# jixinya/EAMM

Measured on AMD Instinct MI355X. Metric: 256x256 frames/sec (dense-motion + generator forward), higher is better.
Workload: dtype f32; 1 GPU; 256x256, 10 keypoints, batch=16 synthetic frames per GPU per step, source encoded once per clip (BASELINE.json configs[2]); parallelism=frame-sharded x1

## Files before the change

eamm_amd/_lib.py:

```python
from __future__ import annotations

import ctypes as C
import os

_HERE = os.path.dirname(os.path.abspath(__file__))
LIB_PATH = os.path.join(_HERE, "libeamm_hip.so")

ABI_VERSION = 6

EAMM_OK = 0
ERR_ARG, ERR_STATE, ERR_KEY, ERR_HIP, ERR_NUMERIC = -1, -2, -3, -4, -5


class EammConfig(C.Structure):
    _fields_ = [
        ("num_channels", C.c_int32), ("num_kp", C.c_int32), ("block_expansion", C.c_int32),
        ("max_features", C.c_int32), ("num_down_blocks", C.c_int32), ("num_bottleneck_blocks", C.c_int32),
        ("estimate_occlusion_map", C.c_int32), ("dm_block_expansion", C.c_int32),
        ("dm_max_features", C.c_int32), ("dm_num_blocks", C.c_int32), ("dm_inv_scale", C.c_int32),
        ("kp_variance", C.c_float), ("height", C.c_int32), ("width", C.c_int32),
        ("max_frames", C.c_int32), ("max_sources", C.c_int32),
    ]


# ... 96 lines not shown
    "eamm_bn_backward_apply": (C.c_int, [C.c_void_p, C.c_void_p, C.c_void_p, C.c_void_p, C.c_int, C.c_int, C.c_int, C.c_void_p,
                                         C.c_void_p]),
    "eamm_bn_apply": (C.c_int, [C.c_void_p, C.c_void_p, C.c_void_p, C.c_void_p, C.c_int, C.c_int, C.c_int, C.c_void_p,
                                C.c_void_p]),
    "eamm_bn_last_error": (C.c_char_p, []),
    "eamm_profile_enable": (C.c_int, [C.c_void_p, C.c_int]),
    "eamm_profile_read": (C.c_int, [C.c_void_p, C.POINTER(C.c_double), C.c_int, C.POINTER(C.c_int64),
                                    C.POINTER(C.c_int64), C.c_int]),
    "eamm_op_conv": (C.c_int, [C.c_int, C.c_void_p, C.c_int, C.c_void_p, C.c_int, C.c_int, C.c_int, C.c_int,
                               C.c_int, C.c_void_p, C.c_void_p, C.c_int, C.c_int, C.c_int, C.c_int, C.c_int, C.c_void_p,
                               C.c_int, C.c_int, C.c_void_p, C.c_int, C.POINTER(C.c_float), C.c_void_p]),
    "eamm_op_conv_ex": (C.c_int, [C.c_int, C.c_void_p, C.c_int, C.c_void_p, C.c_int, C.c_int, C.c_int, C.c_int,
                                  C.c_int, C.c_void_p, C.c_void_p, C.c_int, C.c_int, C.c_int, C.c_int, C.c_int, C.c_void_p,
                                  C.c_int, C.c_int, C.c_void_p, C.c_int, C.POINTER(C.c_float), C.c_void_p, C.c_void_p, C.c_void_p,
                                  C.c_void_p, C.c_void_p, C.c_int, C.c_int, C.c_void_p]),
    "eamm_op_wino_transform": (C.c_int, [C.c_int, C.c_void_p, C.c_void_p, C.c_void_p, C.c_int, C.c_int, C.c_int, C.c_int, C.c_int,
                                         C.c_void_p, C.c_void_p]),
    "eamm_op_warp_ex": (C.c_int, [C.c_int, C.c_void_p, C.c_void_p, C.c_void_p, C.c_int, C.c_int, C.c_int, C.c_int, C.c_int,
                                  C.c_int, C.c_int, C.c_void_p, C.c_int, C.POINTER(C.c_float), C.c_void_p, C.c_void_p, C.c_void_p,
                                  C.c_void_p]),
    "eamm_set_training": (C.c_int, [C.c_void_p, C.c_int]),
    "eamm_train_num_sites": (C.c_int, [C.c_void_p]),
    "eamm_train_site_name": (C.c_char_p, [C.c_void_p, C.c_int]),
    "eamm_train_max_channels": (C.c_int, [C.c_void_p]),
    "eamm_train_begin": (C.c_int, [C.c_void_p, C.c_void_p, C.c_int, C.c_void_p, C.c_void_p, C.c_void_p, C.c_void_p,
                                   C.POINTER(EammBnSite), C.c_int, C.c_float, C.c_float, C.c_int, C.c_void_p, C.POINTER(EammOutputs),
                                   C.c_void_p]),
    "eamm_train_next": (C.c_int, [C.c_void_p, C.POINTER(C.c_int)]),
    "eamm_op_warp": (C.c_int, [C.c_int, C.c_void_p, C.c_void_p, C.c_void_p, C.c_int, C.c_int, C.c_int, C.c_int, C.c_int,
                               C.c_int, C.c_int, C.c_void_p, C.c_int, C.POINTER(C.c_float), C.c_void_p]),
# ... 145 lines not shown
```

eamm_amd/csrc/api_common.h:

```cpp
#pragma once
#include "../../include/eamm_hip.h"
#include "kernels.h"

#include <algorithm>
#include <cmath>
#include <cstdarg>
#include <cstdio>
#include <cstdlib>
#include <cstring>
#include <map>
#include <string>
#include <vector>

namespace eamm {

inline thread_local std::string g_create_error;

namespace {

struct HostTensor {
    std::vector<int64_t> shape;
    std::vector<float> data;
    size_t numel() const {
        size_t n = 1;
// ... 175 lines not shown
    std::copy(b.begin(), b.end(), pad.begin());
    return upload(c, dst, pad);
}

int upload_conv_image(CtxBase* c, float** dst, const HostConv& f, const int* map, int cin_packed, int BN, LayerMode mode,
                      bool swizzle) {
    const bool phase = mode == MODE_PHASE || mode == MODE_PHASES;
    std::vector<float> packed(conv_packed_elems(phase ? 4 : f.kh * f.kw, cin_packed, f.Cout, BN, phase ? 4 : 1));
    if (mode == MODE_PHASES)
        conv_pack_phases_host(f.w.data(), f.Cout, f.Cin, map, cin_packed, BN, swizzle, packed.data());
    else
        conv_pack_host(f.w.data(), f.Cout, f.Cin, f.kh, f.kw, map, cin_packed, BN, phase, swizzle, packed.data());
    return upload(c, dst, packed);
}

int pack_conv(CtxBase* c, const HostConv& f, const int* map, int C0_packed, int C1_packed, LayerMode mode, int dma_cfg,
              ConvLayer* L, int BN = 0) {
    const bool phase = mode == MODE_PHASE || mode == MODE_PHASES;
    L->kh = f.kh;
    L->kw = f.kw;
    L->phase = phase;
    L->C0 = C0_packed;
    L->C1 = C1_packed;
    L->Cout = f.Cout;
    L->BM = 128;
    L->BN = BN ? BN : conv_tile_n(f.Cout);
    L->dma_cfg = dma_cfg;
    if (dma_cfg > 0 && !conv_dma_tile(dma_cfg, &L->BM, &L->BN)) return fail(c, EAMM_ERR_ARG, "unknown dma tile %d", dma_cfg);
    L->ntiles = (f.Cout + L->BN - 1) / L->BN;
    L->nchunks = (phase ? 4 : f.kh * f.kw) * ((C0_packed + C1_packed) / CONV_BK);
// ... 31 lines not shown
    if (tile == 4)
        wino4_pack_host(f.w.data(), f.Cout, f.Cin, L->BN, packed.data());
    else
        wino_pack_host(f.w.data(), f.Cout, f.Cin, L->BN, packed.data());
    if (int rc = upload(c, &L->u, packed)) return rc;
    if (split_planes && tile == 4 && f.Cin % (4 * CONV_BK) == 0) {
        std::vector<float> planes(wino4_split_packed_elems(f.Cout, f.Cin, L->BN));
        wino4_pack_split_host(f.w.data(), f.Cout, f.Cin, L->BN, reinterpret_cast<uint16_t*>(planes.data()));
        if (int rc = upload(c, &L->u3, planes)) return rc;
    }
    return upload_bias(c, &L->bias, f.b, (size_t)L->ntiles * L->BN);
}

int build_layer(CtxBase* c, const std::vector<FoldSpec>& parts, int ks, int C0_real, int C0_packed, int C1_real,
                int C1_packed, ConvLayer* L, LayerMode mode = MODE_PLAIN, std::vector<float>* row_bias = nullptr,
                int dma_cfg = 0, float** w_swizzled = nullptr, int w_swizzled_bn = 0) {
    if (mode != MODE_PLAIN && mode != MODE_ROWSPLIT) return fail(c, EAMM_ERR_ARG, "build_layer: plain or row-split layers only");
    HostConv f;
    if (int rc = fold_conv(c, parts, ks, C0_real + C1_real, &f)) return rc;
    if (mode == MODE_ROWSPLIT) {
        std::vector<float> rb = to_rowsplit(&f);
        if (row_bias) row_bias->swap(rb);
    }
    const std::vector<int> map = channel_map(C0_real, C0_packed, C1_real, C1_packed);
    if (int rc = pack_conv(c, f, map.data(), C0_packed, C1_packed, MODE_PLAIN, dma_cfg, L)) return rc;
    if (!w_swizzled) return EAMM_OK;
    return upload_conv_image(c, w_swizzled, f, map.data(), C0_packed + C1_packed, w_swizzled_bn ? w_swizzled_bn : L->BN,
                             MODE_PLAIN, true);
}

int build_set(CtxBase* c, const std::vector<FoldSpec>& parts, int C0_real, int C0_packed, int C1_real, int C1_packed,
              LayerSet* S, LayerMode mode, bool patch_split_planes = false) {
    HostConv f;
    int rc = fold_conv(c, parts, 3, C0_real + C1_real, &f);
    if (rc) return rc;
    const std::vector<int> map = channel_map(C0_real, C0_packed, C1_real, C1_packed);
    if ((rc = pack_conv(c, f, map.data(), C0_packed, C1_packed, mode, 0, &S->base))) return rc;
    const int Cout = S->base.Cout;
    int cfg = 0;
    if (Cout % 256 == 0) cfg = c->dma_cfg_n256;
// ... 142 lines not shown
```

eamm_amd/csrc/conv_col7.hip:

```cpp
#include "conv_common.h"

#include <algorithm>
#include <cstdlib>

namespace eamm {

typedef __attribute__((address_space(3))) void* lds_ptr_t;

namespace {
constexpr int CT = 16;
constexpr int CPR = CT + 6;
constexpr int CPIX = CPR * CT;
constexpr int CWAVES = 8;
constexpr int CMAXCH = 2;
}

struct Col7Args {
    const float* in;
    unsigned in_bytes, w_bytes;
    int C, B, H, W;
    int tiles_x, tiles_y, tiles;
    const float* w;
    float* out;
    const float* bias;
// ... 328 lines not shown
                static_for<4>([&](auto ic) {
                    constexpr int i = decltype(ic)::value;
                    if (12 * nh + 4 * g + i < PS) dst[4 * g + i] = acc[g][i];
                    acc[g][i] = 0.f;
                });
            });
            __syncthreads();
            col7_gather_tile(p, scratch, Carry, bias_r, b, ty0, tx0, tid);
        }
        asm volatile("s_waitcnt vmcnt(0)" ::: "memory");
        __syncthreads();
        cur = nxt;
    }
}

struct Col7sArgs {
    const float* in0;
    const float* in1;
    unsigned in0_bytes, in1_bytes, w_bytes;
    int C0, C1, B, H, W;
    int tiles_x, tiles_y;
    const float* w;
    float* out;
    int PS;
};

template <int NT>
__global__ __launch_bounds__(CWAVES * 64) void conv_col7s_kernel(const Col7sArgs p) {
    constexpr int BK = CONV_BK;
    constexpr int A_STAGE = CPIX * BK;
// ... 123 lines not shown
    a.W = W;
    a.tiles_x = (W + CT - 1) / CT;
    a.tiles_y = (H + CT - 1) / CT;
    a.w = w_swizzled;
    a.out = out;
    a.PS = pixel_stride;
    constexpr size_t lds = sizeof(float) * (2 * CPIX * CONV_BK + 2 * 3 * 32 * CONV_BK);
    static_assert(lds <= 160 * 1024, "LDS budget");
    static lds_once_mask configured{0};
    if (hipError_t e = ensure_dynamic_lds(conv_col7s_kernel<3>, lds, &configured); e != hipSuccess) return e;
    note_mfma_flops(2.0 * a.tiles_x * a.tiles_y * B * (CT * CT) * 7.0 * (ntile32 * 32) * (C0 + C1));
    hipLaunchKernelGGL(conv_col7s_kernel<3>, dim3(a.tiles_x * a.tiles_y * B), dim3(CWAVES * 64), lds, stream, a);
    return hipGetLastError();
}

static hipError_t col7_launch_impl(const float* in, int C, int B, int H, int W, const float* w_swizzled, float* out, const float* bias,
                                   float* final_out, hipStream_t stream) {
    const bool fused = final_out != nullptr;
    if (C % CONV_BK || C / CONV_BK > CMAXCH || C < CONV_BK) return hipErrorInvalidValue;
    Col7Args a{};
    a.in = in;
    const size_t ib = (size_t)B * H * W * C * 4, wb = (size_t)(C / CONV_BK) * 7 * 32 * CONV_BK * 4;
    if (ib >= 0xFFFFFFF0ull) return hipErrorInvalidValue;
    a.in_bytes = (unsigned)ib;
    a.w_bytes = (unsigned)wb;
    a.C = C;
    a.B = B;
    a.H = H;
    a.W = W;
    a.tiles_x = (W + CT - 1) / CT;
    a.tiles_y = (H + CT - 1) / CT;
    a.tiles = B * a.tiles_x * a.tiles_y;
// ... 6 lines not shown
    a.dbg = dbg;
#else
    a.dbg = 0;
#endif
    const size_t lds = wb + sizeof(float) * (2 * CPIX * CONV_BK + (fused ? 2 * CT * 6 * 21 : 0));
    if (lds > 160 * 1024) return hipErrorInvalidValue;
    static lds_once_mask configured{0}, configured_fused{0};
    if (hipError_t e = fused ? ensure_dynamic_lds(conv_col7_kernel<true>, 160 * 1024, &configured_fused)
                             : ensure_dynamic_lds(conv_col7_kernel<false>, 160 * 1024, &configured);
        e != hipSuccess)
        return e;
    int dev = 0, cus = 256;
    (void)hipGetDevice(&dev);
    (void)hipDeviceGetAttribute(&cus, hipDeviceAttributeMultiprocessorCount, dev);
    const int blocks = std::min(fused ? B * a.tiles_y : a.tiles, cus);
    static const bool mfma4 = knob_int("EAMM_FINAL_MFMA4", 1) != 0;
    if (fused && mfma4) {
        static lds_once_mask configured_q{0};
        note_mfma_flops(2.0 * a.tiles * (CT * CT) * 7.0 * 24 * C);
        if (hipError_t e = ensure_dynamic_lds(conv_col7q_kernel<8>, 160 * 1024, &configured_q); e != hipSuccess) return e;
        hipLaunchKernelGGL(conv_col7q_kernel<8>, dim3(blocks), dim3(CWAVES * 64), lds, stream, a);
        return hipGetLastError();
    }
    note_mfma_flops(2.0 * a.tiles * (CT * CT) * 7.0 * 32 * C);
    if (fused)
        hipLaunchKernelGGL(conv_col7_kernel<true>, dim3(blocks), dim3(CWAVES * 64), lds, stream, a);
    else
        hipLaunchKernelGGL(conv_col7_kernel<false>, dim3(blocks), dim3(CWAVES * 64), lds, stream, a);
    return hipGetLastError();
}

hipError_t conv_col7_launch(const float* in, int C, int B, int H, int W, const float* w_swizzled, float* out,
                            hipStream_t stream) {
    return col7_launch_impl(in, C, B, H, W, w_swizzled, out, nullptr, nullptr, stream);
}

hipError_t conv_col7_fused_launch(const float* in, int C, int B, int H, int W, const float* w_swizzled, const float* bias,
                                  float* out_nchw, hipStream_t stream) {
    if (!bias || !out_nchw) return hipErrorInvalidValue;
    return col7_launch_impl(in, C, B, H, W, w_swizzled, nullptr, bias, out_nchw, stream);
}

}
```

eamm_amd/csrc/eamm_api.hip:

```cpp
#include "eamm_ctx.h"

namespace {

void expected_keys(const eamm_ctx* c, std::vector<std::string>* keys) {
    auto block = [&](const std::string& p) { block_keys(p, keys); };
    const std::string dm = "dense_motion_network.";
    for (int i = 0; i < c->nb; ++i) block(dm + "hourglass.encoder.down_blocks." + std::to_string(i));
    for (int i = 0; i < c->nb; ++i) block(dm + "hourglass.decoder.up_blocks." + std::to_string(i));
    if (c->nb > 0) {
        keys->push_back(dm + "mask.weight");
        keys->push_back(dm + "mask.bias");
        if (c->cfg.estimate_occlusion_map) {
            keys->push_back(dm + "occlusion.weight");
            keys->push_back(dm + "occlusion.bias");
        }
        if (c->cfg.dm_inv_scale != 1) keys->push_back(dm + "down.weight");
    }
    block("first");
    for (int i = 0; i < c->nd; ++i) block("down_blocks." + std::to_string(i));
    for (int i = 0; i < c->nd; ++i) block("up_blocks." + std::to_string(i));
    for (int i = 0; i < c->cfg.num_bottleneck_blocks; ++i) {
        const std::string r = "bottleneck.r" + std::to_string(i);
        for (const char* s : {".conv1.weight", ".conv1.bias", ".conv2.weight", ".conv2.bias", ".norm1.weight",
                              ".norm1.bias", ".norm1.running_mean", ".norm1.running_var", ".norm2.weight",
// ... 378 lines not shown
            if ((rc = build_wino4_rect(c, p + ".conv", p + ".norm", ci, ci, &c->w4down[i]))) return rc;
        }
    }
    c->up.resize(c->nd);
    for (int i = 0; i < c->nd; ++i) {
        const std::string p = "up_blocks." + std::to_string(i);
        const int ci = i == 0 ? c->Cb : c->up_c[i - 1];
        if ((rc = build_set(c, {{p + ".conv", nm(p + ".norm")}}, ci, ci, 0, 0, &c->up[i], MODE_PHASE, true))) return rc;
    }
    if (c->Cimg > 3) {
        if ((rc = build_layer(c, {{"final", ""}}, 7, c->up_c.back(), c->up_c.back(), 0, 0, &c->final_conv))) return rc;
    } else {
        std::vector<float> fb;
        const bool col7_ok = c->col7 && c->up_c.back() % 32 == 0 && c->up_c.back() <= 64;
        if ((rc = build_layer(c, {{"final", ""}}, 7, c->up_c.back(), c->up_c.back(), 0, 0, &c->final_conv,
                              MODE_ROWSPLIT, &fb, 0, col7_ok ? &c->final_w_swz : nullptr)))
            return rc;
        if (c->final_conv.Cout != 21) return fail(c, EAMM_ERR_KEY, "final.weight must have 3 output channels");
        if ((rc = upload(c, &c->final_bias, fb))) return rc;
    }
    {
        std::vector<float> aa((size_t)c->Cpl * 169, 0.f);
        if (g.dm_inv_scale != 1) {
            const HostTensor* t = find(c, dm + "down.weight");
            if (!t || (int)t->numel() != c->Cpl * 169) return fail(c, EAMM_ERR_KEY, "%sdown.weight must be [%d,1,13,13]", dm.c_str(), c->Cimg);
            aa = t->data;
        }
        if ((rc = upload(c, &c->aa_w, aa))) return rc;
    }

    const size_t S = g.max_sources, F = g.max_frames;
// ... 253 lines not shown
```

eamm_amd/csrc/eamm_ctx.h:

```cpp
#pragma once
#include "../../include/eamm_hip.h"
#include "api_common.h"

#include <functional>

using namespace eamm;

struct PassProfile {
    static constexpr int NSTAGE = 22;
    static constexpr int MAXCHAIN = 4;
    static constexpr int NMARK = 8;
    static constexpr int NSUB = 64;
    static constexpr int PROF_CALLS = 256;
    struct Call {
        int n = 0, nchain = 0, sub = 0;
        bool complete = false;
        double flops = 0, flops_bneck = 0, stage_flops[NMARK] = {0};
    };
    bool on = false;
    std::vector<hipEvent_t> events;
    std::vector<hipEvent_t> chain_ev;
    std::vector<Call> calls;
    int used = 0;
    hipEvent_t *ev = nullptr, *cev = nullptr;
// ... 61 lines not shown
    bool wino4_variant_pinned = false;
    int cus = 256;
    float* wino_v = nullptr;
    float* wino_z = nullptr;
    size_t wino_z_elems = 0;
    int wino_min_m = 49152;
    int wino4_min_m = 0;
    std::vector<float*> pre_s, pre_t;
    float* aa_w = nullptr;
    float* head_bias = nullptr;
    int head_nc = 0;
    float* head_w_swz = nullptr;
    float* final_bias = nullptr;
    float* final_part = nullptr;
    float* final_w_swz = nullptr;
    int col7 = 1;
    int final_fused = 1;
    int final_fused_min_rows = 128;
    int head_col7_min_tiles = 128;

    float *feat = nullptr, *src_small = nullptr, *src_full = nullptr;
    float* src_nhwc = nullptr;
    std::vector<float*> enc_tmp;
    float* kp_rec = nullptr;
    int* bad_flag = nullptr;
    float* hg_in = nullptr;
    std::vector<float*> e_buf, u_buf;
    float *logits = nullptr, *deformation = nullptr, *occlusion = nullptr;
    float *xa = nullptr, *xb = nullptr, *act = nullptr, *tmp = nullptr;
    std::vector<float*> up_buf;
// ... 72 lines not shown
```

eamm_amd/csrc/eamm_forward.hip:

```cpp
#include "eamm_ctx.h"
#include <mutex>

namespace {
constexpr int POOL_MAXDEV = 64, POOL_MAXCHAIN = 15;
std::mutex g_pool_mu;
hipStream_t g_pool[POOL_MAXDEV][POOL_MAXCHAIN] = {};
std::mutex g_pool_lease[POOL_MAXDEV];

}

hipStream_t chain_stream(int device, int k) {
    if (device < 0 || device >= POOL_MAXDEV || k < 0 || k >= POOL_MAXCHAIN) return nullptr;
    std::lock_guard<std::mutex> lock(g_pool_mu);
    if (!g_pool[device][k] && hipStreamCreateWithFlags(&g_pool[device][k], hipStreamNonBlocking) != hipSuccess) g_pool[device][k] = nullptr;
    return g_pool[device][k];
}

FrameView make_view(const eamm_ctx* c, int f0, int n, int ns_call, int slab, const float* kd_val, const float* kd_jac,
                    const float* ks_val, const float* ks_jac, const eamm_outputs* o) {
    FrameView v;
    const size_t F = (size_t)f0, K = c->K;
    const size_t HW = (size_t)c->H * c->W, hw = (size_t)c->h * c->w, hwf = (size_t)c->hf * c->wf;
    const size_t sf = ns_call > 1 ? F : 0;
    v.n = n;
// ... 310 lines not shown
}

int stage_final(eamm_ctx* c, const FrameView& v, hipStream_t s) {
    const float* in = v.up_buf[c->nd - 1];
    ConvIO io = conv_for(v, in, c->H, c->W, ACT_NONE, v.final_part);
    if (c->Cimg > 3) {
        io.act = ACT_SIGMOID;
        io.nchw = 1;
        io.out = v.out.prediction;
        HIP_TRY(c, conv_launch(c->final_conv, io, s));
        return EAMM_OK;
    }
    ConvLayer fl = c->final_conv;
    fl.Cout = 32;
    if (final_is_fused(c, v.n)) {
        HIP_TRY(c, conv_col7_fused_launch(in, fl.C0, v.n, c->H, c->W, c->final_w_swz, c->final_bias, v.out.prediction, s));
    } else {
        if (c->final_w_swz && fl.BN == 32)
            HIP_TRY(c, conv_col7_launch(in, fl.C0, v.n, c->H, c->W, c->final_w_swz, v.final_part, s));
        else
            HIP_TRY(c, conv_launch(fl, io, s));
        HIP_TRY(c, final_shift_sum_launch(v.final_part, c->final_bias, v.n, c->H, c->W, v.out.prediction, s));
    }
    if (v.out.frames_u8) HIP_TRY(c, to_u8_launch(v.out.prediction, v.n, c->H, c->W, v.out.frames_u8, s));
    return EAMM_OK;
}

static int forward_view(eamm_ctx* c, const FrameView& v, hipStream_t s, int chain, bool chained) {
    PassProfile& p = c->prof;
    const bool direct = bottleneck_form(c, v.n) == 0;
    int rc;
// ... 217 lines not shown
    return pass_chains(c, n);
}
int eamm_last_stream_set(const eamm_ctx* c) { return c ? c->last_streams : EAMM_ERR_ARG; }
int eamm_describe_plan(const eamm_ctx* c, int n, char* buf, int cap) {
    if (!c || n <= 0 || n > c->cfg.max_frames || !c->finalized) return EAMM_ERR_ARG;
    const int pc = pass_chains(c, n), nk = pc > 1 ? n / pc : n;
    const int form = bottleneck_form(c, nk), bc = pc > 1 ? pc : bottleneck_chains(c, n);
    std::string enc = "[";
    for (int i = 0; i < c->nb; ++i)
        enc += std::string(i ? ", " : "") + (enc_level_wino4(c, i, nk) ? "\"wino4\"" : "\"direct\"");
    enc += "]";
    char tmp[1024];
    const int len = snprintf(tmp, sizeof tmp,
                             "{\"frames\": %d, \"pass_chains\": %d, \"frames_per_chain\": %d, \"bottleneck_form\": %d, \"bottleneck_chains\": %d, "
                             "\"wino4_groups\": %d, \"wino4_variant\": %d, \"hg_encoder\": %s, \"final\": \"%s\", "
                             "\"side_streams\": %d, \"experiments_build\": %d}",
                             n, pc, nk, form, bc, (form == 4 && pc == 1 && bc == 1) ? wino4_groups(c, n) : 1, wino4_variant_for(c, n), enc.c_str(),
                             final_is_fused(c, nk) ? "col7q fused" : "col7 + shift-sum", (int)c->pool_streams.size(),
                             eamm_build_experiments());
    if (buf && cap > 0) {
        const int m = std::min(len, cap - 1);
        std::memcpy(buf, tmp, (size_t)m);
        buf[m] = 0;
    }
    return len;
}

}
```

eamm_amd/csrc/eamm_op_conv.hip:

```cpp
#include "op_common.h"

namespace {

struct ConvOp {
    const float *in0, *in1;
    int C0, C1, B, Hin, Win, up;
    const float *w, *b;
    int Cout, kh, kw, act, pool;
    const float* resid;
    int splitk, tile_n;
    float* out;
    int iters;
    float* avg_ms;
    const float *pre_s, *pre_t;
    float* out2;
    const float *s2, *t2;
    int nchw, split_n;
    const char* name;
    hipStream_t s;
};

const char* conv_refusal(const ConvOp& a) {
    const bool staged = a.tile_n == 0 || a.tile_n == 32 || a.tile_n == 64 || a.tile_n == 128;
    const bool gemm = staged || (a.tile_n > 1000 && a.tile_n <= 1005);
    const bool wino = a.tile_n >= 2000 && a.tile_n < 2200;
    const bool shape_ok = (a.kh == 3 && a.kw == 3) || (a.kh == 7 && a.kw == 7) || (a.kh == 7 && a.kw == 1) ||
                          (a.kh == 1 && a.kw == 1 && staged && !a.up);
    if (!a.in0 || !a.w || !a.b || !a.out || !shape_ok || a.C0 % CONV_BK || a.C1 % CONV_BK || (a.up && (a.kh != 3 || a.kw != 3)))
        return "bad argument";
    if ((a.pre_s != nullptr) != (a.pre_t != nullptr)) return "pre_scale and pre_shift come together";
    if (a.pre_s && !wino) return "pre_scale / pre_shift belong to the Winograd input transform (tile codes 2000, 21xx)";
    const bool second = a.out2 || a.s2 || a.t2;
    if ((second || a.nchw || a.split_n) && !gemm)
        return "out2 / scale2 / shift2 / nchw / split_n belong to the implicit GEMM (tile codes 0, 32, 64, 128, 1001..1005)";
    if (a.split_n < 0 || (a.nchw != 0 && a.nchw != 1)) return "bad nchw / split_n";
    if ((a.s2 != nullptr) != (a.t2 != nullptr) || (a.s2 && !a.out2)) return "scale2 and shift2 come together, with out2";
    if (a.out2 && !a.s2 && a.split_n == 0) return "out2 needs scale2 and shift2";
    if (!op_aligned16(a.pre_s) || !op_aligned16(a.pre_t) || !op_aligned16(a.out2) || !op_aligned16(a.s2) || !op_aligned16(a.t2))
        return "pre_scale, pre_shift, out2, scale2 and shift2 must be 16-byte aligned";
    if (a.pool && (a.resid || a.nchw || a.out2 || a.split_n))
        return "pool does not combine with resid, nchw, out2 or split_n (the pooled epilogue has none of them)";
    if (a.split_n > 0 && (!a.out2 || a.resid || a.nchw || a.Cout <= a.split_n || a.Cout > a.split_n + 4))
        return "split_n needs out2, no resid / pool / nchw, and split_n < Cout <= split_n + 4";
    return nullptr;
}

HostConv op_weights(const ConvOp& a, int Cin, bool with_bias = true) {
    HostConv f;
    f.Cout = a.Cout;
    f.Cin = Cin;
    f.kh = a.kh;
    f.kw = a.kw;
    f.w.assign(a.w, a.w + (size_t)a.Cout * Cin * a.kh * a.kw);
    if (with_bias) f.b.assign(a.b, a.b + a.Cout);
    return f;
}

int op_conv_final(OpBuffers* t, const ConvOp& a) {
    if (a.kh != 7 || a.kw != 7 || a.Cout != 3 || a.act != 2 || a.up || a.pool || a.resid || a.C1 || a.C0 % 32 || a.C0 > 64 || a.C0 < 32)
        return fail(t, EAMM_ERR_ARG, "%s: unsupported fused final-layer configuration", a.name);
    HostConv f = op_weights(a, a.C0);
    const std::vector<float> bias = to_rowsplit(&f);
    float *w = nullptr, *b = nullptr;
    int rc = upload_conv_image(t, &w, f, nullptr, a.C0, conv_tile_n(f.Cout), MODE_PLAIN, true);
    if (rc || (rc = upload(t, &b, bias))) return rc;
    auto fused_final = [&]() { return conv_col7_fused_launch(a.in0, a.C0, a.B, a.Hin, a.Win, w, b, a.out, a.s); };
    HIP_TRY(t, fused_final());
    HIP_TRY(t, time_launches(a.s, a.iters, a.avg_ms, fused_final));
    return EAMM_OK;
}

int op_conv_col7(OpBuffers* t, const ConvOp& a) {
    const bool streamed = a.tile_n == 4001;
    const int bn = streamed ? 96 : 32;
    if (a.kh != 7 || a.kw != 1 || a.up || a.pool || a.resid || a.splitk > 1 || a.Cout != bn || a.act != 0 || a.C0 % 32 || a.C1 % 32 ||
        (!streamed && (a.C1 || a.C0 > 64)))
        return fail(t, EAMM_ERR_ARG, "%s: unsupported column-patch configuration", a.name);
    float* w = nullptr;
    if (int rc = upload_conv_image(t, &w, op_weights(a, a.C0 + a.C1, false), nullptr, a.C0 + a.C1, bn, MODE_PLAIN, true)) return rc;
    auto col7 = [&]() {
        return streamed ? conv_col7s_launch(a.in0, a.C0, a.in1, a.C1, a.B, a.Hin, a.Win, w, 3, a.out, 96, a.s)
// ... 72 lines not shown
    io.resid = a.resid;
    io.nchw = a.nchw;
    io.out2 = a.out2;
    io.s2 = a.s2;
    io.t2 = a.t2;
    io.split_n = a.split_n;
    if (io.partial_cap && (rc = dev_alloc(t, &io.partial, io.partial_cap))) return rc;
    auto gemm = [&]() { return conv_launch(L, io, a.s, a.splitk); };
    HIP_TRY(t, gemm());
    HIP_TRY(t, time_launches(a.s, a.iters, a.avg_ms, gemm));
    return EAMM_OK;
}

int op_conv_run(OpBuffers* t, const ConvOp& a) {
    int rc;
    if (a.tile_n == 4002) rc = op_conv_final(t, a);
    else if (a.tile_n == 4000 || a.tile_n == 4001) rc = op_conv_col7(t, a);
    else if (a.tile_n == 3000 || a.tile_n == 3003 || a.tile_n == 3004) rc = op_conv_patch(t, a);
    else if (a.tile_n >= 2000 && a.tile_n < 2200) rc = op_conv_wino(t, a);
    else rc = op_conv_gemm(t, a);
    if (rc) return rc;
    HIP_TRY(t, hipStreamSynchronize(a.s));
    return EAMM_OK;
}

int op_conv_call(int device, ConvOp a, void* stream_) {
    if (const char* why = conv_refusal(a)) return fail(nullptr, EAMM_ERR_ARG, "%s: %s", a.name, why);
    DeviceGuard guard(device);
    if (guard.status != hipSuccess) return fail(nullptr, EAMM_ERR_HIP, "hipSetDevice failed");
    a.s = reinterpret_cast<hipStream_t>(stream_);
    OpBuffers t(device, a.s);
// ... 29 lines not shown
    return op_conv_call(device,
                        ConvOp{in0, in1, C0, C1, B, Hin, Win, up, w_host, b_host, Cout, kh, kw, act, pool, resid, splitk, tile_n, out, iters,
                               avg_ms, pre_scale, pre_shift, out2, scale2, shift2, nchw, split_n, "eamm_op_conv_ex", nullptr},
                        stream_);
}

int eamm_op_conv(int device, const float* in0, int C0, const float* in1, int C1, int B, int Hin, int Win, int up,
                 const float* w_host, const float* b_host, int Cout, int kh, int kw, int act, int pool,
                 const float* resid, int splitk, int tile_n, float* out, int iters, float* avg_ms, void* stream_) {
    return op_conv_call(device,
                        ConvOp{in0, in1, C0, C1, B, Hin, Win, up, w_host, b_host, Cout, kh, kw, act, pool, resid, splitk, tile_n, out, iters,
                               avg_ms, nullptr, nullptr, nullptr, nullptr, nullptr, 0, 0, "eamm_op_conv", nullptr},
                        stream_);
}

int eamm_op_wino_transform(int device, const float* x, const float* scale, const float* shift, int B, int H, int W, int C, int tile,
                           float* V, void* stream_) {
    const bool tile_ok = tile == 2 || tile == 4;
    OP_ENTRY(!x || !V || !tile_ok || B < 1 || H < 1 || W < 1 || C < 1 || H % tile || W % tile || (C & 3) ||
                 (scale != nullptr) != (shift != nullptr) || !op_aligned16(x) || !op_aligned16(V) || !op_aligned16(scale) ||
                 !op_aligned16(shift) || !op_count_ok((tile + 2) * (tile + 2), (long long)B * (H / tile) * (W / tile), C),
             "eamm_op_wino_transform: bad argument");
    OP_DONE(tile == 4 ? wino4_transform_launch(x, scale, shift, B, H, W, C, V, s) : wino_transform_launch(x, scale, shift, B, H, W, C, V, s),
            "eamm_op_wino_transform");
}

int eamm_op_warp_ex(int device, const float* feat, const float* deformation, const float* occlusion, int n, int ns, int hf, int wf, int C,
                    int h, int w, float* out, int iters, float* avg_ms, float* out2, const float* scale2, const float* shift2,
                    void* stream_) {
    return op_warp_call("eamm_op_warp_ex", device, feat, deformation, occlusion, n, ns, hf, wf, C, h, w, out, out2, scale2, shift2, iters,
// ... 11 lines not shown
```

eamm_amd/csrc/kernels.h:

```cpp
#pragma once
#include <hip/hip_runtime.h>
#include <stddef.h>
#include <stdint.h>

namespace eamm {

constexpr int CONV_BK = 32;
constexpr int CONV_LDK = CONV_BK + 4;
inline size_t round64(size_t n) { return (n + 63) / 64 * 64; }
constexpr int KP_STRIDE = 8;

enum Act { ACT_NONE = 0, ACT_RELU = 1, ACT_SIGMOID = 2 };

void note_mfma_flops(double flops);
double take_mfma_flops();
double total_mfma_flops();

long long knob_int(const char* name, long long dflt);
int knobs_json(char* buf, int cap);

struct ConvArgs {
    const float* in0;
    const float* in1;
    int C0, C1;
// ... 68 lines not shown
size_t patch_packed_elems(int Cin_packed, int Cout);
size_t patch_poly_packed_elems(int Cin_packed, int Cout);
void patch_poly_pack_host(const float* w_oihw_3x3, int Cout, int Cin, const int* cin_map, int cin_packed, float* dst);
size_t patch_poly_split_packed_elems(int Cin_packed, int Cout);
void patch_poly_pack_split_host(const float* w_oihw_3x3, int Cout, int Cin, const int* cin_map, int cin_packed, uint16_t* dst);
hipError_t patch_poly_launch(const PatchLayer& L, const float* in0, const float* in1, int B, int H, int W, int act,
                             float* out, hipStream_t stream, int splits = 1, float* partial = nullptr, size_t partial_cap = 0);
int patch_poly_splits(const PatchLayer& L, int B, int H, int W, int max_splits, int cus);
void patch_pack_host(const float* w_oihw_3x3, int Cout, int Cin, const int* cin_map, int cin_packed, float* dst);
hipError_t patch_phase_launch(const PatchLayer& L, const float* in0, const float* in1, int B, int H, int W, int act,
                              float* out, hipStream_t stream);

hipError_t conv_col7_launch(const float* in, int C, int B, int H, int W, const float* w_swizzled, float* out,
                            hipStream_t stream);
hipError_t conv_col7_fused_launch(const float* in, int C, int B, int H, int W, const float* w_swizzled, const float* bias,
                                  float* out_nchw, hipStream_t stream);

hipError_t conv_col7s_launch(const float* in0, int C0, const float* in1, int C1, int B, int H, int W, const float* w_swizzled,
                             int ntile32, float* out, int pixel_stride, hipStream_t stream);

struct WinoLayer {
    int Cin = 0, Cout = 0, BN = 128, ntiles = 0;
    int tile = 2;
    float* u = nullptr;
    float* u3 = nullptr;
    float* bias = nullptr;
};
size_t wino_packed_elems(int Cout, int Cin, int BN);
void wino_pack_host(const float* w_oihw, int Cout, int Cin, int BN, float* dst);
hipError_t wino_transform_launch(const float* x, const float* s, const float* t, int B, int H, int W, int C, float* V,
                                 hipStream_t stream);
// ... 233 lines not shown
```

include/eamm_hip.h:

```cpp
#ifndef EAMM_HIP_H_
#define EAMM_HIP_H_

#include <stddef.h>
#include <stdint.h>

#ifdef __cplusplus
extern "C" {
#endif

#define EAMM_ABI_VERSION 6

typedef enum eamm_status {
    EAMM_OK = 0,
    EAMM_ERR_ARG = -1,
    EAMM_ERR_STATE = -2,
    EAMM_ERR_KEY = -3,
    EAMM_ERR_HIP = -4,
    EAMM_ERR_NUMERIC = -5
} eamm_status;

typedef struct eamm_ctx eamm_ctx;

typedef struct eamm_config {
    int32_t num_channels;
// ... 202 lines not shown
#define EAMM_NSTAGE 22
int eamm_profile_enable(eamm_ctx* ctx, int on);
int eamm_profile_read(eamm_ctx* ctx, double* stage_ms, int nstage, int64_t* calls, int64_t* frames, int reset);


int eamm_op_conv(int device, const float* in0, int C0, const float* in1, int C1, int B, int Hin, int Win, int up,
                 const float* weight_host, const float* bias_host, int Cout, int kh, int kw,
                 int act, int pool, const float* resid, int splitk, int tile_n, float* out, int iters,
                 float* avg_ms, void* stream);

int eamm_op_conv_ex(int device, const float* in0, int C0, const float* in1, int C1, int B, int Hin, int Win, int up,
                    const float* weight_host, const float* bias_host, int Cout, int kh, int kw,
                    int act, int pool, const float* resid, int splitk, int tile_n, float* out, int iters,
                    float* avg_ms, const float* pre_scale, const float* pre_shift, float* out2, const float* scale2,
                    const float* shift2, int nchw, int split_n, void* stream);

int eamm_op_wino_transform(int device, const float* x, const float* scale, const float* shift, int B, int H, int W, int C, int tile,
                           float* V, void* stream);

int eamm_op_one_euro(int device, const float* x, int T, int E, float mincutoff, float beta, float dcutoff, float freq, float scale,
                     float* out, float* state, int resume, void* stream);

int64_t eamm_op_mfcc_frames(int64_t n_samples, int pad);
int eamm_op_mfcc(int device, const float* pcm, int64_t n_samples, int n_clips, int64_t clip_stride, int pad, float* out, void* stream);

int eamm_op_resize_aa(int device, const uint8_t* in, int n, int H, int W, int C, const double* taps_y, int ry, const double* taps_x,
                      int rx, uint8_t* out, void* stream);
int eamm_op_similarity_warp(int device, const uint8_t* in, int n, int H, int W, int C, const double* maps, int mode, void* out,
                            void* stream);
int eamm_op_emotion_augment(int device, const float* aligned, int64_t n_src, int64_t t0, int count, int flip, const double* rot,
// ... 127 lines not shown
```

Before: 4391 frames/s.

## Run fused final 7x7 conv on split-bf16 MFMA with pre-split weight planes

```diff
diff --git a/eamm_amd/_lib.py b/eamm_amd/_lib.py
--- a/eamm_amd/_lib.py
+++ b/eamm_amd/_lib.py
@@ -134,6 +134,8 @@
                                   C.c_int, C.c_void_p, C.c_void_p, C.c_int, C.c_int, C.c_int, C.c_int, C.c_int, C.c_void_p,
                                   C.c_int, C.c_int, C.c_void_p, C.c_int, C.POINTER(C.c_float), C.c_void_p, C.c_void_p, C.c_void_p,
                                   C.c_void_p, C.c_void_p, C.c_int, C.c_int, C.c_void_p]),
+    "eamm_final_split_planes_elems": (C.c_size_t, [C.c_int]),
+    "eamm_final_split_planes": (C.c_int, [C.c_void_p, C.c_int, C.c_void_p, C.c_void_p]),
     "eamm_op_wino_transform": (C.c_int, [C.c_int, C.c_void_p, C.c_void_p, C.c_void_p, C.c_int, C.c_int, C.c_int, C.c_int, C.c_int,
                                          C.c_void_p, C.c_void_p]),
     "eamm_op_warp_ex": (C.c_int, [C.c_int, C.c_void_p, C.c_void_p, C.c_void_p, C.c_int, C.c_int, C.c_int, C.c_int, C.c_int,
diff --git a/eamm_amd/csrc/api_common.h b/eamm_amd/csrc/api_common.h
--- a/eamm_amd/csrc/api_common.h
+++ b/eamm_amd/csrc/api_common.h
@@ -213,6 +213,12 @@
     return upload(c, dst, packed);
 }
 
+int upload_col7_split(CtxBase* c, float** dst, const HostConv& f, const int* map, int cin_packed) {
+    std::vector<float> planes(col7_split_packed_elems(cin_packed));
+    col7_pack_split_host(f.w.data(), f.Cout, f.Cin, map, cin_packed, reinterpret_cast<uint16_t*>(planes.data()));
+    return upload(c, dst, planes);
+}
+
 int pack_conv(CtxBase* c, const HostConv& f, const int* map, int C0_packed, int C1_packed, LayerMode mode, int dma_cfg,
               ConvLayer* L, int BN = 0) {
     const bool phase = mode == MODE_PHASE || mode == MODE_PHASES;
@@ -274,7 +280,7 @@
 
 int build_layer(CtxBase* c, const std::vector<FoldSpec>& parts, int ks, int C0_real, int C0_packed, int C1_real,
                 int C1_packed, ConvLayer* L, LayerMode mode = MODE_PLAIN, std::vector<float>* row_bias = nullptr,
-                int dma_cfg = 0, float** w_swizzled = nullptr, int w_swizzled_bn = 0) {
+                int dma_cfg = 0, float** w_swizzled = nullptr, int w_swizzled_bn = 0, float** w_col7_split = nullptr) {
     if (mode != MODE_PLAIN && mode != MODE_ROWSPLIT) return fail(c, EAMM_ERR_ARG, "build_layer: plain or row-split layers only");
     HostConv f;
     if (int rc = fold_conv(c, parts, ks, C0_real + C1_real, &f)) return rc;
@@ -284,6 +290,8 @@
     }
     const std::vector<int> map = channel_map(C0_real, C0_packed, C1_real, C1_packed);
     if (int rc = pack_conv(c, f, map.data(), C0_packed, C1_packed, MODE_PLAIN, dma_cfg, L)) return rc;
+    if (w_col7_split)
+        if (int rc = upload_col7_split(c, w_col7_split, f, map.data(), C0_packed + C1_packed)) return rc;
     if (!w_swizzled) return EAMM_OK;
     return upload_conv_image(c, w_swizzled, f, map.data(), C0_packed + C1_packed, w_swizzled_bn ? w_swizzled_bn : L->BN,
                              MODE_PLAIN, true);
diff --git a/eamm_amd/csrc/conv_col7.hip b/eamm_amd/csrc/conv_col7.hip
--- a/eamm_amd/csrc/conv_col7.hip
+++ b/eamm_amd/csrc/conv_col7.hip
@@ -2,6 +2,7 @@
 
 #include <algorithm>
 #include <cstdlib>
+#include <cstring>
 
 namespace eamm {
 
@@ -366,6 +367,146 @@
     }
 }
 
+namespace {
+constexpr int SG = 16;
+constexpr int S_WBLK = 2 * PS * 16;
+constexpr int S_WGROUP = 7 * 3 * S_WBLK;
+constexpr int S_WBYTES = (CMAXCH * 2 * S_WGROUP + 1023) / 1024 * 1024;
+constexpr int S_ROWS = CPR;
+constexpr int S_F32 = S_ROWS * 1024;
+constexpr int S_OCT = CPIX * 16;
+constexpr int S_PLANE = 2 * S_OCT;
+constexpr int S_PSTAGE = 3 * S_PLANE;
+constexpr int S_LDS = S_WBYTES + S_F32 + 2 * S_PSTAGE + 2 * CARRY * 4;
+static_assert(S_LDS <= 160 * 1024, "LDS budget");
+static_assert(CT * CT * PS * 4 <= S_PSTAGE, "the tile's partial products fit a consumed plane stage");
+static_assert(CPR <= 3 * CWAVES, "at most three pieces per wave");
+}
+
+__global__ __launch_bounds__(CWAVES * 64) void conv_col7b_kernel(const Col7Args p) {
+    extern __shared__ __attribute__((aligned(16))) float smem[];
+    char* const Ws = reinterpret_cast<char*>(smem);
+    char* const Fs = Ws + S_WBYTES;
+    char* const Ps = Fs + S_F32;
+    float* const Carry = reinterpret_cast<float*>(Ps + 2 * S_PSTAGE);
+    const int groups = p.C / SG;
+
+    const int tid = threadIdx.x;
+    const int lane = tid & 63;
+    const int wave = __builtin_amdgcn_readfirstlane(tid >> 6);
+    const int l31 = lane & 31, half = lane >> 5;
+
+    const __amdgpu_buffer_rsrc_t rsi = __builtin_amdgcn_make_buffer_rsrc((void*)p.in, 0, p.in_bytes, 0x00020000);
+    const __amdgpu_buffer_rsrc_t rsw = __builtin_amdgcn_make_buffer_rsrc((void*)p.w, 0, p.w_bytes, 0x00020000);
+    constexpr unsigned OOB = 0xFFFFFFF0u;
+
+    const int first = blockIdx.x;
+    const int items = p.B * p.tiles_y;
+    const int my_items = first < items ? (items - first + (int)gridDim.x - 1) / (int)gridDim.x : 0;
+    const int units = my_items * p.tiles_x * groups;
+    if (units == 0) return;
+
+    const int d_px = lane & 15;
+    const int d_rel = d_px * p.C + 8 * ((lane >> 4) & 1) + 4 * (lane >> 5);
+    auto dma_patch_piece = [&](auto ic, const Col7Pos& pos) {
+        constexpr int i = decltype(ic)::value;
+        const int j = wave + CWAVES * i;
+        const int y = pos.ty0 + j - 3, x = pos.tx0 + d_px;
+        const bool ok = ((unsigned)y < (unsigned)p.H) & ((unsigned)x < (unsigned)p.W);
+        const int base = ((pos.b * p.H + y) * p.W + pos.tx0) * p.C + pos.cc * SG;
+        const unsigned off = ok ? (unsigned)(base + d_rel) * 4u : OOB;
+        __builtin_amdgcn_raw_ptr_buffer_load_lds(rsi, (lds_ptr_t)(Fs + j * 1024), 16, off, 0, 0, 0);
+    };
+    auto split_pieces = [&](char* dst) {
+        static_for<2>([&](auto rc) {
+            constexpr int r = decltype(rc)::value;
+            const int j = r == 0 ? wave + CWAVES * half : wave + 2 * CWAVES;
+            if (r == 0 || (half == 0 && j < S_ROWS)) {
+                const char* src = Fs + j * 1024 + l31 * 16;
+                const f32x4 x0 = *reinterpret_cast<const f32x4*>(src), x1 = *reinterpret_cast<const f32x4*>(src + 512);
+                u32x4 pl[3];
+                wino4_split3(x0, x1, pl);
+                char* d = dst + (l31 >> 4) * S_OCT + (j * CT + (l31 & 15)) * 16;
+                static_for<3>([&](auto kc) { *reinterpret_cast<u32x4*>(d + decltype(kc)::value * S_PLANE) = pl[decltype(kc)::value]; });
+            }
+        });
+    };
+
+    for (int j = wave; j < groups * S_WGROUP / 1024 + 1; j += CWAVES)
+        if (j * 1024 < (int)p.w_bytes)
+            __builtin_amdgcn_raw_ptr_buffer_load_lds(rsw, (lds_ptr_t)(Ws + j * 1024), 16, (unsigned)(j * 1024 + lane * 16), 0, 0, 0);
+    Col7Pos cur{0, 0, first, 0, 0, 0};
+    col7_pos_decode<true>(cur, p);
+    static_for<3>([&](auto ic) {
+        if (wave + CWAVES * decltype(ic)::value < S_ROWS) dma_patch_piece(ic, cur);
+    });
+    asm volatile("s_waitcnt vmcnt(0)" ::: "memory");
+    split_pieces(Ps);
+    __syncthreads();
+
+    f32x16 acc;
+    static_for<16>([&](auto rc) { acc[decltype(rc)::value] = 0.f; });
+    const int a_off = half * S_OCT + (32 * wave + l31) * 16;
+    const int b_off = half * (PS * 16) + min(l31, PS - 1) * 16;
+    const float bias_r[3] = {p.bias[0], p.bias[1], p.bias[2]};
+
+    for (int u = 0; u < units; ++u) {
+        const int st = u & 1;
+        const bool more = u + 1 < units;
+        const int b = cur.b, ty0 = cur.ty0, tx0 = cur.tx0, cc = cur.cc;
+        Col7Pos nxt = cur;
+        col7_pos_next<true>(nxt, p, groups, (int)gridDim.x);
+        const char* a_stage = Ps + st * S_PSTAGE + a_off;
+        const char* w_stage = Ws + cc * S_WGROUP + b_off;
+        u32x4 ap[2][3], wp[2][3];
+        auto fetch = [&](auto tc, int buf) {
+            constexpr int t = decltype(tc)::value;
+            static_for<3>([&](auto kc) {
+                constexpr int k = decltype(kc)::value;
+                ap[buf][k] = *reinterpret_cast<const u32x4*>(a_stage + k * S_PLANE + t * (CT * 16));
+                wp[buf][k] = *reinterpret_cast<const u32x4*>(w_stage + (t * 3 + k) * S_WBLK);
+            });
+        };
+        fetch(std::integral_constant<int, 0>{}, 0);
+        static_for<7>([&](auto tc) {
+            constexpr int t = decltype(tc)::value;
+            if constexpr (t + 1 < 7) fetch(std::integral_constant<int, t + 1>{}, (t + 1) & 1);
+            __builtin_amdgcn_sched_barrier(0);
+            static_for<6>([&](auto mc) {
+                constexpr int m = decltype(mc)::value;
+                constexpr int pa = m == 0 ? 0 : m == 1 ? 2 : m == 2 ? 1 : m == 3 ? 0 : m == 4 ? 1 : 0;
+                constexpr int pb = m == 0 ? 2 : m <= 3 ? 0 : 1;
+                acc = __builtin_amdgcn_mfma_f32_32x32x16_bf16(__builtin_bit_cast(bf16x8_t, ap[t & 1][pa]),
+                                                              __builtin_bit_cast(bf16x8_t, wp[t & 1][pb]), acc, 0, 0, 0);
+            });
+            if constexpr (t < 3) {
+                __builtin_amdgcn_sched_barrier(0);
+                if (more && wave + CWAVES * t < S_ROWS) dma_patch_piece(tc, nxt);
+            }
+            __builtin_amdgcn_sched_barrier(0);
+        });
+        if (more) {
+            asm volatile("s_waitcnt vmcnt(0)" ::: "memory");
+            split_pieces(Ps + (st ^ 1) * S_PSTAGE);
+        }
+        if (cc == groups - 1) {
+            __syncthreads();
+            float* const scratch = reinterpret_cast<float*>(Ps + st * S_PSTAGE);
+            static_for<16>([&](auto rc) {
+                constexpr int r = decltype(rc)::value;
+                const int m = (r & 3) + 8 * (r >> 2) + 4 * half;
+                const int row = 2 * wave + (m >> 4), col = m & 15;
+                if (l31 < PS) scratch[(row * CT + col) * PS + l31] = acc[r];
+                acc[r] = 0.f;
+            });
+            __syncthreads();
+            col7_gather_tile(p, scratch, Carry, bias_r, b, ty0, tx0, tid);
+        }
+        __syncthreads();
+        cur = nxt;
+    }
+}
+
 struct Col7sArgs {
     const float* in0;
     const float* in1;
@@ -519,8 +660,31 @@
     return hipGetLastError();
 }
 
+size_t col7_split_packed_elems(int cin_packed) { return ((size_t)(cin_packed / SG) * S_WGROUP + 1023) / 1024 * 256; }
+
+void col7_pack_split_host(const float* w, int Cout, int Cin, const int* cin_map, int cin_packed, uint16_t* dst) {
+    const size_t total = 2 * col7_split_packed_elems(cin_packed);
+    for (size_t i = 0; i < total; ++i) dst[i] = 0;
+    auto bits = [](float f) { uint32_t b; memcpy(&b, &f, 4); return b; };
+    auto top = [](uint32_t b) { b &= 0xFFFF0000u; float f; memcpy(&f, &b, 4); return f; };
+    for (int n = 0; n < Cout && n < PS; ++n)
+        for (int cp = 0; cp < cin_packed; ++cp) {
+            const int c = cin_map ? cin_map[cp] : cp;
+            if (c < 0 || c >= Cin) continue;
+            for (int t = 0; t < 7; ++t) {
+                const float u = w[((size_t)n * Cin + c) * 7 + t];
+                const float r = u - top(bits(u)), r2 = r - top(bits(r));
+                const int g = cp / SG, h = (cp % SG) >> 3, e = cp & 7;
+                uint16_t* blk = dst + ((size_t)(g * 7 + t) * 3 * S_WBLK + h * (PS * 16) + n * 16) / 2 + e;
+                blk[0] = (uint16_t)(bits(u) >> 16);
+                blk[S_WBLK / 2] = (uint16_t)(bits(r) >> 16);
+                blk[S_WBLK] = (uint16_t)(bits(r2) >> 16);
+            }
+        }
+}
+
 static hipError_t col7_launch_impl(const float* in, int C, int B, int H, int W, const float* w_swizzled, float* out, const float* bias,
-                                   float* final_out, hipStream_t stream) {
+                                   float* final_out, hipStream_t stream, const float* w_split = nullptr) {
     const bool fused = final_out != nullptr;
     if (C % CONV_BK || C / CONV_BK > CMAXCH || C < CONV_BK) return hipErrorInvalidValue;
     Col7Args a{};
@@ -557,6 +721,15 @@
     (void)hipGetDevice(&dev);
     (void)hipDeviceGetAttribute(&cus, hipDeviceAttributeMultiprocessorCount, dev);
     const int blocks = std::min(fused ? B * a.tiles_y : a.tiles, cus);
+    if (fused && w_split) {
+        static lds_once_mask configured_b{0};
+        a.w = w_split;
+        a.w_bytes = (unsigned)(col7_split_packed_elems(C) * 4);
+        note_mfma_flops(2.0 * a.tiles * (CT * CT) * 7.0 * 24 * C);
+        if (hipError_t e = ensure_dynamic_lds(conv_col7b_kernel, S_LDS, &configured_b); e != hipSuccess) return e;
+        hipLaunchKernelGGL(conv_col7b_kernel, dim3(blocks), dim3(CWAVES * 64), S_LDS, stream, a);
+        return hipGetLastError();
+    }
     static const bool mfma4 = knob_int("EAMM_FINAL_MFMA4", 1) != 0;
     if (fused && mfma4) {
         static lds_once_mask configured_q{0};
@@ -579,9 +752,9 @@
 }
 
 hipError_t conv_col7_fused_launch(const float* in, int C, int B, int H, int W, const float* w_swizzled, const float* bias,
-                                  float* out_nchw, hipStream_t stream) {
+                                  float* out_nchw, hipStream_t stream, const float* w_split) {
     if (!bias || !out_nchw) return hipErrorInvalidValue;
-    return col7_launch_impl(in, C, B, H, W, w_swizzled, nullptr, bias, out_nchw, stream);
-}
-
-}
+    return col7_launch_impl(in, C, B, H, W, w_swizzled, nullptr, bias, out_nchw, stream, w_split);
+}
+
+}
diff --git a/eamm_amd/csrc/eamm_api.hip b/eamm_amd/csrc/eamm_api.hip
--- a/eamm_amd/csrc/eamm_api.hip
+++ b/eamm_amd/csrc/eamm_api.hip
@@ -416,7 +416,7 @@
         std::vector<float> fb;
         const bool col7_ok = c->col7 && c->up_c.back() % 32 == 0 && c->up_c.back() <= 64;
         if ((rc = build_layer(c, {{"final", ""}}, 7, c->up_c.back(), c->up_c.back(), 0, 0, &c->final_conv,
-                              MODE_ROWSPLIT, &fb, 0, col7_ok ? &c->final_w_swz : nullptr)))
+                              MODE_ROWSPLIT, &fb, 0, col7_ok ? &c->final_w_swz : nullptr, 0, col7_ok ? &c->final_w3 : nullptr)))
             return rc;
         if (c->final_conv.Cout != 21) return fail(c, EAMM_ERR_KEY, "final.weight must have 3 output channels");
         if ((rc = upload(c, &c->final_bias, fb))) return rc;
diff --git a/eamm_amd/csrc/eamm_ctx.h b/eamm_amd/csrc/eamm_ctx.h
--- a/eamm_amd/csrc/eamm_ctx.h
+++ b/eamm_amd/csrc/eamm_ctx.h
@@ -99,6 +99,7 @@
     float* final_bias = nullptr;
     float* final_part = nullptr;
     float* final_w_swz = nullptr;
+    float* final_w3 = nullptr;
     int col7 = 1;
     int final_fused = 1;
     int final_fused_min_rows = 128;
diff --git a/eamm_amd/csrc/eamm_forward.hip b/eamm_amd/csrc/eamm_forward.hip
--- a/eamm_amd/csrc/eamm_forward.hip
+++ b/eamm_amd/csrc/eamm_forward.hip
@@ -348,7 +348,7 @@
     ConvLayer fl = c->final_conv;
     fl.Cout = 32;
     if (final_is_fused(c, v.n)) {
-        HIP_TRY(c, conv_col7_fused_launch(in, fl.C0, v.n, c->H, c->W, c->final_w_swz, c->final_bias, v.out.prediction, s));
+        HIP_TRY(c, conv_col7_fused_launch(in, fl.C0, v.n, c->H, c->W, c->final_w_swz, c->final_bias, v.out.prediction, s, c->final_w3));
     } else {
         if (c->final_w_swz && fl.BN == 32)
             HIP_TRY(c, conv_col7_launch(in, fl.C0, v.n, c->H, c->W, c->final_w_swz, v.final_part, s));
@@ -596,9 +596,10 @@
     const int len = snprintf(tmp, sizeof tmp,
                              "{\"frames\": %d, \"pass_chains\": %d, \"frames_per_chain\": %d, \"bottleneck_form\": %d, \"bottleneck_chains\": %d, "
                              "\"wino4_groups\": %d, \"wino4_variant\": %d, \"hg_encoder\": %s, \"final\": \"%s\", "
-                             "\"side_streams\": %d, \"experiments_build\": %d}",
+                             "\"final_products\": \"%s\", \"side_streams\": %d, \"experiments_build\": %d}",
                              n, pc, nk, form, bc, (form == 4 && pc == 1 && bc == 1) ? wino4_groups(c, n) : 1, wino4_variant_for(c, n), enc.c_str(),
-                             final_is_fused(c, nk) ? "col7q fused" : "col7 + shift-sum", (int)c->pool_streams.size(),
+                             final_is_fused(c, nk) ? "col7q fused" : "col7 + shift-sum",
+                             final_is_fused(c, nk) && c->final_w3 ? "split-bf16" : "fp32", (int)c->pool_streams.size(),
                              eamm_build_experiments());
     if (buf && cap > 0) {
         const int m = std::min(len, cap - 1);
diff --git a/eamm_amd/csrc/eamm_op_conv.hip b/eamm_amd/csrc/eamm_op_conv.hip
--- a/eamm_amd/csrc/eamm_op_conv.hip
+++ b/eamm_amd/csrc/eamm_op_conv.hip
@@ -28,6 +28,10 @@
                           (a.kh == 1 && a.kw == 1 && staged && !a.up);
     if (!a.in0 || !a.w || !a.b || !a.out || !shape_ok || a.C0 % CONV_BK || a.C1 % CONV_BK || (a.up && (a.kh != 3 || a.kw != 3)))
         return "bad argument";
+    if ((a.tile_n == 4002 || a.tile_n == 4003) &&
+        (a.kh != 7 || a.kw != 7 || a.Cout != 3 || a.act != 2 || a.up || a.pool || a.resid || a.C1 || a.C0 % 32 || a.C0 > 64 || a.C0 < 32))
+        return a.tile_n == 4002 ? "unsupported fused final-layer configuration (tile code 4002)"
+                                : "unsupported fused final-layer configuration (tile code 4003)";
     if ((a.pre_s != nullptr) != (a.pre_t != nullptr)) return "pre_scale and pre_shift come together";
     if (a.pre_s && !wino) return "pre_scale / pre_shift belong to the Winograd input transform (tile codes 2000, 21xx)";
     const bool second = a.out2 || a.s2 || a.t2;
@@ -57,14 +61,12 @@
 }
 
 int op_conv_final(OpBuffers* t, const ConvOp& a) {
-    if (a.kh != 7 || a.kw != 7 || a.Cout != 3 || a.act != 2 || a.up || a.pool || a.resid || a.C1 || a.C0 % 32 || a.C0 > 64 || a.C0 < 32)
-        return fail(t, EAMM_ERR_ARG, "%s: unsupported fused final-layer configuration", a.name);
     HostConv f = op_weights(a, a.C0);
     const std::vector<float> bias = to_rowsplit(&f);
-    float *w = nullptr, *b = nullptr;
+    float *w = nullptr, *b = nullptr, *w3 = nullptr;
     int rc = upload_conv_image(t, &w, f, nullptr, a.C0, conv_tile_n(f.Cout), MODE_PLAIN, true);
-    if (rc || (rc = upload(t, &b, bias))) return rc;
-    auto fused_final = [&]() { return conv_col7_fused_launch(a.in0, a.C0, a.B, a.Hin, a.Win, w, b, a.out, a.s); };
+    if (rc || (rc = upload(t, &b, bias)) || (a.tile_n == 4002 && (rc = upload_col7_split(t, &w3, f, nullptr, a.C0)))) return rc;
+    auto fused_final = [&]() { return conv_col7_fused_launch(a.in0, a.C0, a.B, a.Hin, a.Win, w, b, a.out, a.s, w3); };
     HIP_TRY(t, fused_final());
     HIP_TRY(t, time_launches(a.s, a.iters, a.avg_ms, fused_final));
     return EAMM_OK;
@@ -167,7 +169,7 @@
 
 int op_conv_run(OpBuffers* t, const ConvOp& a) {
     int rc;
-    if (a.tile_n == 4002) rc = op_conv_final(t, a);
+    if (a.tile_n == 4002 || a.tile_n == 4003) rc = op_conv_final(t, a);
     else if (a.tile_n == 4000 || a.tile_n == 4001) rc = op_conv_col7(t, a);
     else if (a.tile_n == 3000 || a.tile_n == 3003 || a.tile_n == 3004) rc = op_conv_patch(t, a);
     else if (a.tile_n >= 2000 && a.tile_n < 2200) rc = op_conv_wino(t, a);
@@ -227,6 +229,22 @@
                         stream_);
 }
 
+size_t eamm_final_split_planes_elems(int C) { return (C == 32 || C == 64) ? 2 * col7_split_packed_elems(C) : 0; }
+int eamm_final_split_planes(const float* w_host, int C, float* rowsplit, uint16_t* planes) {
+    if (!w_host || !rowsplit || !planes || (C != 32 && C != 64))
+        return fail(nullptr, EAMM_ERR_ARG, "eamm_final_split_planes: bad argument (C = 32 | 64)");
+    HostConv f;
+    f.Cout = 3;
+    f.Cin = C;
+    f.kh = f.kw = 7;
+    f.w.assign(w_host, w_host + (size_t)3 * C * 49);
+    f.b.assign(3, 0.f);
+    to_rowsplit(&f);
+    std::copy(f.w.begin(), f.w.end(), rowsplit);
+    col7_pack_split_host(f.w.data(), f.Cout, f.Cin, nullptr, C, planes);
+    return EAMM_OK;
+}
+
 int eamm_op_wino_transform(int device, const float* x, const float* scale, const float* shift, int B, int H, int W, int C, int tile,
                            float* V, void* stream_) {
     const bool tile_ok = tile == 2 || tile == 4;
diff --git a/eamm_amd/csrc/kernels.h b/eamm_amd/csrc/kernels.h
--- a/eamm_amd/csrc/kernels.h
+++ b/eamm_amd/csrc/kernels.h
@@ -106,7 +106,9 @@
 hipError_t conv_col7_launch(const float* in, int C, int B, int H, int W, const float* w_swizzled, float* out,
                             hipStream_t stream);
 hipError_t conv_col7_fused_launch(const float* in, int C, int B, int H, int W, const float* w_swizzled, const float* bias,
-                                  float* out_nchw, hipStream_t stream);
+                                  float* out_nchw, hipStream_t stream, const float* w_split = nullptr);
+size_t col7_split_packed_elems(int cin_packed);
+void col7_pack_split_host(const float* w_rowsplit, int Cout, int Cin, const int* cin_map, int cin_packed, uint16_t* dst);
 
 hipError_t conv_col7s_launch(const float* in0, int C0, const float* in1, int C1, int B, int H, int W, const float* w_swizzled,
                              int ntile32, float* out, int pixel_stride, hipStream_t stream);
diff --git a/include/eamm_hip.h b/include/eamm_hip.h
--- a/include/eamm_hip.h
+++ b/include/eamm_hip.h
@@ -240,6 +240,9 @@
                     int act, int pool, const float* resid, int splitk, int tile_n, float* out, int iters,
                     float* avg_ms, const float* pre_scale, const float* pre_shift, float* out2, const float* scale2,
                     const float* shift2, int nchw, int split_n, void* stream);
+
+size_t eamm_final_split_planes_elems(int C);
+int eamm_final_split_planes(const float* weight_host, int C, float* rowsplit, uint16_t* planes);
 
 int eamm_op_wino_transform(int device, const float* x, const float* scale, const float* shift, int B, int H, int W, int C, int tile,
                            float* V, void* stream);
```

Result: faster. 4449 frames/s, median of 6 (+1.3%).
